# aticejiang/MLAgg-UNet

Hardware: AMD Instinct MI355X
Metric: images/sec (train step) MLAgg-UNet-2D 256x256 bs10 (higher is better)
Workload: dtype f32; 1 GPU; nnUNetTrainer_MLAgg_2D_dt_MS train step, AbdomenMRI-shaped 256x256x1, 14 classes, attention variant B (BASELINE.json configs[1]); batch_per_gpu=10, global_batch=10, parallelism=dp1, launch=eager, miopen=tuned find-db (mlagg-unet_amd/miopen_db), library_gemm=TunableOp table (mlagg-unet_amd/gemm_db), tuning off

## Files before the change

### mlagg-unet_amd/csrc/api.hip

```cpp
#include <hip/hip_runtime.h>

#include <mutex>
#include <vector>

#include "mlagg_hip.h"
#include "prof.h"

namespace mlagg_prof {

int g_selected = -1;

namespace {
struct Rec {
    int id;
    hipEvent_t start, stop;
};
std::mutex g_mu;
std::vector<Rec> g_recs;
size_t g_used = 0;
const char *const kNames[K_COUNT] = {
    "selscan_fwd_kernel<false>", "selscan_chunk_prefix", "selscan_fwd_kernel<true>", "selscan_bwd_local_kernel",
    "selscan_bwd_group_kernel", "selscan_reduce_partials", "local_attn_fwd_kernel", "local_attn_bwd_a_kernel",
    "local_attn_bwd_b_kernel", "pooled_attn_fwd_kernel", "pooled_attn_bwd1_kernel",
    "pooled_attn_bwd2_kernel", "dwconv_tiled_kernel<fwd>", "dwconv_tiled_kernel<dgrad>", "dwconv_bwd_weight_kernel", "linear weight gradient (K5w: linear_wgrad_kernel / linear_wgrad_x3_kernel + reduce)", "layernorm_fwd_kernel",
    "layernorm_bwd_kernel", "dwconv_nchw_fwd_kernel", "dwconv_nchw_bwd (data+weight+reduce)",
    "cross_scan_kernel<false>", "cross_scan_kernel<true>", "gate_fwd_kernel", "gate_bwd_kernel",
    "linear forward + data gradient (K5: linear_x3_kernel on weight images; MLAGG_K5_V2=0: linear_lp_kernel<true, MODE> / linear_mfma_kernel<true>)", "linear data gradient (K5: linear_mfma_kernel<false> / linear_lp_kernel<false, MODE>)", "row_scale_kernel", "dice_ce_stats_kernel", "dice_ce_grad_kernel", "transpose_tile_kernel", "bias gradient (plane_sum / column_sum)", "plane_norm_fwd_kernel", "plane_norm_bwd_kernel", "adamw (sumsq + update)", "flash_fwd_kernel", "flash_bwd (dq + dk/dv)", "channel_epilogue (bias + residual + GELU)",
    "sel1_fwd_kernel<2, false>", "sel1_fwd_kernel<2, true>", "sel1_bwd_local_kernel<2>", "sel1_bwd_kernel<2>",
    "sel1_fwd_kernel<R != 2, false>", "sel1_fwd_kernel<R != 2, true>", "sel1_bwd_local_kernel<R != 2>", "sel1_bwd_kernel<R != 2>",
    "sel1_prefix_kernel", "sel1 reductions (step partials + per-chunk rows)",
    "volume_pad_kernel (+ guard fill)", "conv_wgrad_taps_kernel", "conv_wgrad_reduce_kernel", "conv_taps_kernel (forward / data gradient)",
    "gelu_pool (forward + backward)", "conv1x1 (forward / data gradient / weight gradient)",
    "conv3x3 (forward / data gradient / weight gradient, incl. weight image and reduce)",
    "tok_fwd_kernel<false>", "tok_fwd_kernel<true>", "tok_bwd_local_kernel", "tok_bwd_group_kernel",
    "sw_gather_kernel", "sw_fold_kernel", "sw_finalize_kernel", "resample_linear_kernel", "export_kernel",
    "pp_box_kernel", "pp_stats_kernel (+ final)", "pp_normalize_kernel", "pp_minmax_kernel", "pp_cubic_kernel", "pp_gather_kernel",
    "cc_local_kernel", "cc_merge_kernel", "cc_compress_kernel", "cc_size_kernel", "cc_max_kernel", "cc_write_kernel",
    "sf_stats_kernel (+ init)", "sf_codes_kernel", "sf_zpass_kernel", "sf_ypass_kernel", "sf_xpass_kernel", "sf_sum_kernel",
    "aug3d_resample_kernel", "pt_seg_crop_kernel", "pt_seg_resize_kernel", "pt_rank_count_kernel (+ scan)", "pt_rank_select_kernel",
    "cl_local_kernel", "cl_merge_kernel", "cl_compress_kernel", "cl_flag_kernel", "cl_scan (count + offsets + apply)", "cl_rewrite_kernel",
    "cl_overlap_kernel", "cl_match_kernel", "ens_mean_kernel", "label_confusion_kernel", "dice_bce_stats_kernel", "dice_bce_grad_kernel",
    "aug3d_planar_kernel", "sw_gather_onehot_kernel"};
}

void record(int id, hipStream_t st, bool begin)
{
    std::lock_guard<std::mutex> lk(g_mu);
    if (begin) {
        if (g_used == g_recs.size()) {
            Rec r{id, nullptr, nullptr};
            if (hipEventCreate(&r.start) != hipSuccess || hipEventCreate(&r.stop) != hipSuccess) return;
            g_recs.push_back(r);
        }
        g_recs[g_used].id = id;
        (void)hipEventRecord(g_recs[g_used].start, st);
        ++g_used;
    } else if (g_used > 0) {
        (void)hipEventRecord(g_recs[g_used - 1].stop, st);
    }
}

}

extern "C" const char *mlagg_version(void) { return "mlagg_hip 0.1 (gfx950)"; }

extern "C" const char *mlagg_error_string(int code)
{
    switch (code) {
    case 0: return "success";
    case MLAGG_E_UNSUPPORTED: return "unsupported shape for the gfx950 kernels";
    case MLAGG_E_NULLPTR: return "required pointer argument is NULL";
    case MLAGG_E_WORKSPACE: return "workspace too small";
    default: return code > 0 ? hipGetErrorString(static_cast<hipError_t>(code)) : "unknown mlagg error";
    }
}

extern "C" int mlagg_profile_kernel_count(void) { return mlagg_prof::K_COUNT; }

extern "C" const char *mlagg_profile_kernel_name(int id)
{
    return (id >= 0 && id < mlagg_prof::K_COUNT) ? mlagg_prof::kNames[id] : "?";
}

extern "C" int mlagg_profile_select(int id)
{
    if (id < -2 || id >= mlagg_prof::K_COUNT) return MLAGG_E_UNSUPPORTED;
    mlagg_prof::g_selected = id;
    return 0;
}

extern "C" int mlagg_profile_collect(double *ms, int *counts)
{
    using namespace mlagg_prof;
    if (!ms || !counts) return MLAGG_E_NULLPTR;
    std::lock_guard<std::mutex> lk(g_mu);
    for (int i = 0; i < K_COUNT; ++i) { ms[i] = 0.0; counts[i] = 0; }
    for (size_t i = 0; i < g_used; ++i) {
        float t = 0.f;
        if (hipEventSynchronize(g_recs[i].stop) != hipSuccess) continue;
        if (hipEventElapsedTime(&t, g_recs[i].start, g_recs[i].stop) != hipSuccess) continue;
        ms[g_recs[i].id] += t;
        counts[g_recs[i].id] += 1;
    }
    g_used = 0;
    return 0;
}
```

### mlagg-unet_amd/csrc/local_attn.hip

```cpp
#include <hip/hip_runtime.h>

#include "mlagg_hip.h"
#include "prof.h"
#include "internal.h"
#include "reduce.h"

namespace {

constexpr int HD2 = 48;
constexpr int PER = 12;
constexpr int TILE = 8;
constexpr float RMS_EPS = 1e-5f;
constexpr float OUT_GAIN = 0.2f;
constexpr int WS_PER_UNIT = 76;

struct Geom {
    int batch, H, W, nh, d;
    int q_stride, kv_stride, out_stride;
    float scale;
};

__device__ __forceinline__ void load12(const float *__restrict__ p, float (&x)[PER])
{
    const float4 a = *reinterpret_cast<const float4 *>(p);
    const float4 b = *reinterpret_cast<const float4 *>(p + 4);
    const float4 c = *reinterpret_cast<const float4 *>(p + 8);
    x[0] = a.x; x[1] = a.y; x[2] = a.z; x[3] = a.w;
    x[4] = b.x; x[5] = b.y; x[6] = b.z; x[7] = b.w;
    x[8] = c.x; x[9] = c.y; x[10] = c.z; x[11] = c.w;
}

__device__ __forceinline__ void store12(float *__restrict__ p, const float (&x)[PER])
{
    *reinterpret_cast<float4 *>(p) = make_float4(x[0], x[1], x[2], x[3]);
    *reinterpret_cast<float4 *>(p + 4) = make_float4(x[4], x[5], x[6], x[7]);
    *reinterpret_cast<float4 *>(p + 8) = make_float4(x[8], x[9], x[10], x[11]);
}

struct Unit {
    int b, h, y, x, r;
    bool act;
};

__device__ __forceinline__ Unit unit_id(const Geom &g)
{
    Unit u;
    const int tiles_x = (g.W + TILE - 1) / TILE;
    const int ty = blockIdx.x / tiles_x, tx = blockIdx.x - ty * tiles_x;
    const int lu = threadIdx.x >> 2;
    u.r = threadIdx.x & 3;
    u.y = ty * TILE + (lu >> 3);
    u.x = tx * TILE + (lu & 7);
    u.h = blockIdx.y;
    u.b = blockIdx.z;
    u.act = u.y < g.H && u.x < g.W;
    return u;
}

__device__ __forceinline__ void window_softmax(const float (&l)[9], unsigned valid, float (&s)[9])
{
    float m = -3.0e38f;
#pragma unroll
    for (int j = 0; j < 9; ++j)
        if ((valid >> j) & 1) m = fmaxf(m, l[j]);
    float z = 0.f;
#pragma unroll
    for (int j = 0; j < 9; ++j) {
        s[j] = ((valid >> j) & 1) ? __expf(l[j] - m) : 0.f;
        z += s[j];
    }
    const float iz = 1.f / z;
#pragma unroll
    for (int j = 0; j < 9; ++j) s[j] *= iz;
}

struct Front {
    float s[9];
    float other[9];
    float Aw[9];
    float o[PER];
    float rstd;
    unsigned valid;
};

__device__ __forceinline__ void front_half(const Geom &g, const Unit &u, const float *__restrict__ q,
                                           const float *__restrict__ kv, float lam, Front &f)
{
    const int N = g.H * g.W;
    const size_t tok = (size_t)u.b * N + (size_t)u.y * g.W + u.x;
    float qv[PER];
    load12(q + tok * g.q_stride + u.h * HD2 + PER * u.r, qv);
    float lg[9];
    f.valid = 0;
#pragma unroll
    for (int j = 0; j < 9; ++j) {
        const int yy = u.y + j / 3 - 1, xx = u.x + j % 3 - 1;
        const bool in = yy >= 0 && yy < g.H && xx >= 0 && xx < g.W;
        float p = 0.f;
        if (in) {
            f.valid |= 1u << j;
            float kx[PER];
            load12(kv + ((size_t)u.b * N + (size_t)yy * g.W + xx) * g.kv_stride + u.h * HD2 + PER * u.r, kx);
#pragma unroll
            for (int e = 0; e < PER; ++e) p += qv[e] * kx[e];
        }
        lg[j] = (p + dpp_quad_xor1(p)) * g.scale;
    }
    window_softmax(lg, f.valid, f.s);
#pragma unroll
    for (int j = 0; j < 9; ++j) {
        f.other[j] = dpp_quad_xor2(f.s[j]);
        f.Aw[j] = u.r < 2 ? f.s[j] - lam * f.other[j] : f.other[j] - lam * f.s[j];
    }
#pragma unroll
    for (int e = 0; e < PER; ++e) f.o[e] = 0.f;
}

__device__ __forceinline__ void stage_lepe(float (*swt)[HD2], const float *__restrict__ lepe_w, int head)
{
    for (int i = threadIdx.x; i < 9 * HD2; i += blockDim.x) {
        const int c = i / 9, j = i - 9 * c;
        swt[j][c] = lepe_w[(head * HD2 + c) * 9 + j];
    }
    __syncthreads();
}

__global__ void __launch_bounds__(256)
local_attn_fwd_kernel(const float *__restrict__ q, const float *__restrict__ kv, const float *__restrict__ lamp,
                      const float *__restrict__ subln_w, const float *__restrict__ lepe_w,
                      const float *__restrict__ lepe_b, float *__restrict__ out, Geom g)
{
    __shared__ float swt[9][HD2];
    stage_lepe(swt, lepe_w, blockIdx.y);
    const Unit u = unit_id(g);
    if (!u.act) return;
    const float lam = lamp[0];
    const int N = g.H * g.W;
    Front f;
    front_half(g, u, q, kv, lam, f);
    const int cbase = u.h * HD2 + PER * u.r;
    float lp[PER];
#pragma unroll
    for (int e = 0; e < PER; ++e) lp[e] = lepe_b[cbase + e];
#pragma unroll
    for (int j = 0; j < 9; ++j) {
        if (!((f.valid >> j) & 1)) continue;
        const int yy = u.y + j / 3 - 1, xx = u.x + j % 3 - 1;
        float vx[PER], wj[PER];
        load12(kv + ((size_t)u.b * N + (size_t)yy * g.W + xx) * g.kv_stride + g.d + cbase, vx);
        load12(&swt[j][PER * u.r], wj);
#pragma unroll
        for (int e = 0; e < PER; ++e) {
            f.o[e] += f.Aw[j] * vx[e];
            lp[e] += wj[e] * vx[e];
        }
    }
    float ss = 0.f;
#pragma unroll
    for (int e = 0; e < PER; ++e) ss += f.o[e] * f.o[e];
    const float rstd = rsqrtf(quad_sum(ss) * (1.f / HD2) + RMS_EPS);
    float res[PER];
#pragma unroll
    for (int e = 0; e < PER; ++e) res[e] = OUT_GAIN * subln_w[PER * u.r + e] * f.o[e] * rstd + lp[e];
    store12(out + ((size_t)u.b * N + (size_t)u.y * g.W + u.x) * g.out_stride + cbase, res);
}

__global__ void __launch_bounds__(256)
local_attn_bwd_a_kernel(const float *__restrict__ q, const float *__restrict__ kv, const float *__restrict__ lamp,
                        const float *__restrict__ subln_w, const float *__restrict__ dout, int dout_stride,
                        float *__restrict__ dq, int dq_stride, float *__restrict__ ws, float *__restrict__ pgrad, Geom g)
{
    __shared__ float red[4][4][PER + 1];
    __syncthreads();
    const Unit u = unit_id(g);
    const float lam = lamp[0];
    const int N = g.H * g.W;
    float dw[PER];
#pragma unroll
    for (int e = 0; e < PER; ++e) dw[e] = 0.f;
    float dl_acc = 0.f;
    if (u.act) {
        Front f;
        front_half(g, u, q, kv, lam, f);
        const int cbase = u.h * HD2 + PER * u.r;
        const size_t tok = (size_t)u.b * N + (size_t)u.y * g.W + u.x;
        float vj[9][PER];
#pragma unroll
        for (int j = 0; j < 9; ++j) {
            const int yy = u.y + j / 3 - 1, xx = u.x + j % 3 - 1;
            if ((f.valid >> j) & 1) {
                load12(kv + ((size_t)u.b * N + (size_t)yy * g.W + xx) * g.kv_stride + g.d + cbase, vj[j]);
            } else {
#pragma unroll
                for (int e = 0; e < PER; ++e) vj[j][e] = 0.f;
            }
#pragma unroll
            for (int e = 0; e < PER; ++e) f.o[e] += f.Aw[j] * vj[j][e];
        }
        float ss = 0.f;
#pragma unroll
        for (int e = 0; e < PER; ++e) ss += f.o[e] * f.o[e];
        const float rstd = rsqrtf(quad_sum(ss) * (1.f / HD2) + RMS_EPS);
        float dy[PER], dO[PER];
        load12(dout + tok * dout_stride + cbase, dy);
        float dot = 0.f;
#pragma unroll
        for (int e = 0; e < PER; ++e) {
            const float wdy = subln_w[PER * u.r + e] * dy[e];
            dot += wdy * f.o[e];
            dw[e] = OUT_GAIN * dy[e] * f.o[e] * rstd;
        }
        dot = quad_sum(dot) * (1.f / HD2) * rstd * rstd;
#pragma unroll
        for (int e = 0; e < PER; ++e)
            dO[e] = OUT_GAIN * rstd * (subln_w[PER * u.r + e] * dy[e] - f.o[e] * dot);
        float dA[9];
#pragma unroll
        for (int j = 0; j < 9; ++j) {
            float p = 0.f;
#pragma unroll
            for (int e = 0; e < PER; ++e) p += dO[e] * vj[j][e];
            dA[j] = quad_sum(p);
        }
        float dsum = 0.f, dlm = 0.f;
        float ds[9];
#pragma unroll
        for (int j = 0; j < 9; ++j) {
            ds[j] = u.r < 2 ? dA[j] : -lam * dA[j];
            dsum += ds[j] * f.s[j];
            if (u.r == 2) dlm -= dA[j] * f.s[j];
        }
        dl_acc = dlm;
        float dlg[9];
#pragma unroll
        for (int j = 0; j < 9; ++j) dlg[j] = f.s[j] * (ds[j] - dsum) * g.scale;
        float dqv[PER];
#pragma unroll
        for (int e = 0; e < PER; ++e) dqv[e] = 0.f;
#pragma unroll
        for (int j = 0; j < 9; ++j) {
            if (!((f.valid >> j) & 1)) continue;
            const int yy = u.y + j / 3 - 1, xx = u.x + j % 3 - 1;
            float kx[PER];
            load12(kv + ((size_t)u.b * N + (size_t)yy * g.W + xx) * g.kv_stride + u.h * HD2 + PER * u.r, kx);
#pragma unroll
            for (int e = 0; e < PER; ++e) dqv[e] += dlg[j] * kx[e];
        }
        store12(dq + tok * dq_stride + cbase, dqv);
        float *wrow = ws + (tok * g.nh + u.h) * WS_PER_UNIT;
        if (u.r == 0) {
#pragma unroll
            for (int j = 0; j < 9; ++j) { wrow[j] = f.Aw[j]; wrow[9 + j] = dlg[j]; }
        }
        if (u.r == 2) {
#pragma unroll
            for (int j = 0; j < 9; ++j) wrow[18 + j] = dlg[j];
        }
        store12(wrow + 28 + PER * u.r, dO);
    }
#pragma unroll
    for (int e = 0; e < PER; ++e) {
        float v = dw[e];
#pragma unroll
        for (int off = 4; off < 64; off <<= 1) v += __shfl_xor(v, off, 64);
        if ((threadIdx.x & 63) < 4) red[threadIdx.x >> 6][threadIdx.x & 3][e] = v;
    }
    {
        float v = dl_acc;
#pragma unroll
        for (int off = 1; off < 64; off <<= 1) v += __shfl_xor(v, off, 64);
        if ((threadIdx.x & 63) == 0) red[threadIdx.x >> 6][0][PER] = v;
    }
    __syncthreads();
    float *prow = pgrad + ((size_t)(blockIdx.z * gridDim.y + blockIdx.y) * gridDim.x + blockIdx.x) * (4 * PER + 1);
    if (threadIdx.x < 4 * PER) {
        const int r = threadIdx.x / PER, e = threadIdx.x % PER;
        prow[threadIdx.x] = (red[0][r][e] + red[1][r][e]) + (red[2][r][e] + red[3][r][e]);
    }
    if (threadIdx.x == 63) prow[4 * PER] = (red[0][0][PER] + red[1][0][PER]) + (red[2][0][PER] + red[3][0][PER]);
}

__global__ void __launch_bounds__(256)
local_attn_bwd_b_kernel(const float *__restrict__ q, const float *__restrict__ lepe_w,
                        const float *__restrict__ dout, int dout_stride, const float *__restrict__ ws,
                        float *__restrict__ dkv, int dkv_stride, Geom g)
{
    __shared__ float swt[9][HD2];
    stage_lepe(swt, lepe_w, blockIdx.y);
    const Unit u = unit_id(g);
    if (!u.act) return;
    const int N = g.H * g.W;
    const int cbase = u.h * HD2 + PER * u.r;
    const size_t tok = (size_t)u.b * N + (size_t)u.y * g.W + u.x;
    float dk[PER], dv[PER];
#pragma unroll
    for (int e = 0; e < PER; ++e) { dk[e] = 0.f; dv[e] = 0.f; }
#pragma unroll
    for (int jj = 0; jj < 9; ++jj) {
        const int yy = u.y + jj / 3 - 1, xx = u.x + jj % 3 - 1;
        if (!(yy >= 0 && yy < g.H && xx >= 0 && xx < g.W)) continue;
        const int jw = 8 - jj;
        const size_t ti = (size_t)u.b * N + (size_t)yy * g.W + xx;
        const float *wrow = ws + (ti * g.nh + u.h) * WS_PER_UNIT;
        const float Ai = wrow[jw];
        const float dli = wrow[(u.r < 2 ? 9 : 18) + jw];
        float dOi[PER], qi[PER], dyi[PER], wj[PER];
        load12(wrow + 28 + PER * u.r, dOi);
        load12(q + ti * g.q_stride + cbase, qi);
        load12(dout + ti * dout_stride + cbase, dyi);
        load12(&swt[jw][PER * u.r], wj);
#pragma unroll
        for (int e = 0; e < PER; ++e) {
            dv[e] += Ai * dOi[e] + wj[e] * dyi[e];
            dk[e] += dli * qi[e];
        }
    }
    store12(dkv + tok * dkv_stride + cbase, dk);
    store12(dkv + tok * dkv_stride + g.d + cbase, dv);
}

int make_geom(Geom &g, int batch, int H, int W, int nh, int qs, int kvs, int outs, float scale)
{
    if (batch <= 0 || H <= 0 || W <= 0 || nh <= 0 || batch > 65535 || nh > 65535) return MLAGG_E_UNSUPPORTED;
    g.batch = batch; g.H = H; g.W = W; g.nh = nh; g.d = nh * HD2;
    g.q_stride = qs; g.kv_stride = kvs; g.out_stride = outs; g.scale = scale;
    if (qs < g.d || kvs < 2 * g.d || (qs & 3) || (kvs & 3)) return MLAGG_E_UNSUPPORTED;
    return 0;
}

dim3 tile_grid(const Geom &g)
{
    return dim3(((g.W + TILE - 1) / TILE) * ((g.H + TILE - 1) / TILE), g.nh, g.batch);
}

}

extern "C" int mlagg_local_attn_fwd(const float *q, int q_stride, const float *kv, int kv_stride,
                                    const float *lam, const float *subln_w, const float *lepe_w,
                                    const float *lepe_b, float *out, int out_stride, int batch, int H, int W,
                                    int nh, float scale, void *stream)
{
    if (!q || !kv || !lam || !subln_w || !lepe_w || !lepe_b || !out) return MLAGG_E_NULLPTR;
    Geom g;
    if (int rc = make_geom(g, batch, H, W, nh, q_stride, kv_stride, out_stride, scale)) return rc;
    if (out_stride < g.d || (out_stride & 3)) return MLAGG_E_UNSUPPORTED;
    hipStream_t st = static_cast<hipStream_t>(stream);
    { MLAGG_TIMED(K_LOCAL_FWD, st); hipLaunchKernelGGL(local_attn_fwd_kernel, tile_grid(g), dim3(256), 0, st, q, kv, lam, subln_w, lepe_w, lepe_b,
                       out, g); }
    return (int)hipGetLastError();
}

extern "C" size_t mlagg_local_attn_bwd_workspace_floats(int batch, int H, int W, int nh)
{
    const size_t tiles = (size_t)((W + TILE - 1) / TILE) * ((H + TILE - 1) / TILE) * nh * batch;
    return (size_t)batch * H * W * nh * WS_PER_UNIT + mlagg_internal::dwconv_wgrad_workspace_floats(batch, H, W, nh * HD2) +
           tiles * (4 * PER + 1);
}

extern "C" int mlagg_local_attn_bwd(const float *q, int q_stride, const float *kv, int kv_stride,
                                    const float *lam, const float *subln_w, const float *lepe_w,
                                    const float *dout, int dout_stride, float *dq, int dq_stride, float *dkv,
                                    int dkv_stride, float *dlam, float *dsubln_w, float *dlepe_w,
                                    float *dlepe_b, float *workspace, int batch, int H, int W, int nh,
                                    float scale, void *stream)
{
    if (!q || !kv || !lam || !subln_w || !lepe_w || !dout || !dq || !dkv || !dlam || !dsubln_w || !dlepe_w ||
        !dlepe_b || !workspace)
        return MLAGG_E_NULLPTR;
    Geom g;
    if (int rc = make_geom(g, batch, H, W, nh, q_stride, kv_stride, dout_stride, scale)) return rc;
    if (dout_stride < g.d || (dout_stride & 3) || dq_stride < g.d || (dq_stride & 3) || dkv_stride < 2 * g.d ||
        (dkv_stride & 3))
        return MLAGG_E_UNSUPPORTED;
    hipStream_t st = static_cast<hipStream_t>(stream);
    const dim3 tg = tile_grid(g);
    const int nwg = (int)(tg.x * tg.y * tg.z);
    float *pgrad = workspace + (size_t)batch * H * W * nh * WS_PER_UNIT + mlagg_internal::dwconv_wgrad_workspace_floats(batch, H, W, g.d);
    { MLAGG_TIMED(K_LOCAL_BWD_A, st); hipLaunchKernelGGL(local_attn_bwd_a_kernel, tg, dim3(256), 0, st, q, kv, lam, subln_w, dout,
                       dout_stride, dq, dq_stride, workspace, pgrad, g);
      hipLaunchKernelGGL(mlagg_internal::column_sum_split_kernel<0>, dim3(1), dim3(1024), 0, st, pgrad, nwg, 4 * PER + 1, 4 * PER + 1,
                         4 * PER, dsubln_w, dlam); }
    { MLAGG_TIMED(K_LOCAL_BWD_B, st); hipLaunchKernelGGL(local_attn_bwd_b_kernel, tile_grid(g), dim3(256), 0, st, q, lepe_w, dout, dout_stride,
                       workspace, dkv, dkv_stride, g); }
    mlagg_internal::dwconv_wgrad_launch(kv + g.d, kv_stride, dout, dout_stride, nullptr, dlepe_w, dlepe_b,
                                        workspace + (size_t)batch * H * W * nh * WS_PER_UNIT, batch, H, W, g.d, 0, st);
    return (int)hipGetLastError();
}
```

### mlagg-unet_amd/csrc/prof.h

```cpp
#pragma once
#include <hip/hip_runtime.h>

namespace mlagg_prof {

enum KernelId {
    K_SELSCAN_FWD_LOCAL = 0, K_SELSCAN_PREFIX, K_SELSCAN_FWD_FINAL, K_SELSCAN_BWD_LOCAL, K_SELSCAN_BWD,
    K_SELSCAN_REDUCE, K_LOCAL_FWD, K_LOCAL_BWD_A, K_LOCAL_BWD_B, K_POOLED_FWD,
    K_POOLED_BWD1, K_POOLED_BWD2, K_DWCONV_FWD, K_DWCONV_BWD_DATA, K_DWCONV_BWD_WEIGHT, K_LINEAR_WGRAD, K_LAYERNORM_FWD, K_LAYERNORM_BWD, K_DWCONV_NCHW_FWD, K_DWCONV_NCHW_BWD, K_CROSS_SCAN, K_CROSS_MERGE, K_GATE_FWD, K_GATE_BWD, K_LINEAR_FWD, K_LINEAR_DGRAD, K_ROW_SCALE, K_LOSS_STATS, K_LOSS_GRAD, K_TRANSPOSE, K_BIAS_GRAD, K_PLANE_NORM_FWD, K_PLANE_NORM_BWD, K_ADAMW, K_FLASH_FWD, K_FLASH_BWD, K_CHANNEL_EPI,
    K_SEL1_FWD_LOCAL_R2, K_SEL1_FWD_FINAL_R2, K_SEL1_BWD_LOCAL_R2, K_SEL1_BWD_R2, K_SEL1_FWD_LOCAL, K_SEL1_FWD_FINAL, K_SEL1_BWD_LOCAL,
    K_SEL1_BWD, K_SEL1_PREFIX, K_SEL1_REDUCE, K_CONV_PAD, K_CONV_WGRAD, K_CONV_WGRAD_REDUCE, K_CONV_TAPS, K_GELU_POOL, K_CONV1X1, K_CONV3X3, K_TOK_FWD_LOCAL, K_TOK_FWD_FINAL, K_TOK_BWD_LOCAL, K_TOK_BWD_GROUP, K_SW_GATHER, K_SW_FOLD, K_SW_FINALIZE, K_RESAMPLE_LINEAR, K_EXPORT_SEG, K_PP_BOX, K_PP_STATS, K_PP_NORMALIZE, K_PP_MINMAX, K_PP_CUBIC, K_PP_GATHER, K_CC_LOCAL, K_CC_MERGE, K_CC_COMPRESS, K_CC_SIZE, K_CC_MAX, K_CC_WRITE, K_SF_STATS, K_SF_CODES, K_SF_ZPASS, K_SF_YPASS, K_SF_XPASS, K_SF_SUM, K_AUG3D_RESAMPLE, K_PT_SEG_CROP, K_PT_SEG_RESIZE, K_PT_RANK_COUNTS, K_PT_RANK_SELECT,
    K_CL_LOCAL, K_CL_MERGE, K_CL_COMPRESS, K_CL_FLAG, K_CL_SCAN, K_CL_REWRITE, K_CL_OVERLAP, K_CL_MATCH,
    K_ENS_MEAN, K_LABEL_CONFUSION, K_REGION_LOSS_STATS, K_REGION_LOSS_GRAD, K_AUG3D_PLANAR, K_SW_GATHER_ONEHOT, K_COUNT
};

extern int g_selected;
void record(int id, hipStream_t st, bool begin);

struct Scope {
    int id;
    hipStream_t st;
    bool on;
    Scope(int id_, hipStream_t st_) : id(id_), st(st_), on(g_selected == -2 || g_selected == id_)
    {
        if (on) record(id, st, true);
    }
    ~Scope()
    {
        if (on) record(id, st, false);
    }
};

}

#define MLAGG_TIMED(id, st) mlagg_prof::Scope mlagg_prof_scope_##id(mlagg_prof::id, st)
```

### mlagg-unet_amd/profiling.py

```python
import ctypes

from . import _lib


def _names():
    lib = _lib.lib()
    return [lib.mlagg_profile_kernel_name(i).decode() for i in range(lib.mlagg_profile_kernel_count())]


def select_all():
    _lib.check(_lib.lib().mlagg_profile_select(-2), "mlagg_profile_select")


def select(name):
    idx = -1 if name is None else _names().index(name)
    _lib.check(_lib.lib().mlagg_profile_select(idx), "mlagg_profile_select")


def collect():
    lib = _lib.lib()
    n = lib.mlagg_profile_kernel_count()
    ms = (ctypes.c_double * n)()
    cnt = (ctypes.c_int * n)()
    _lib.check(lib.mlagg_profile_collect(ms, cnt), "mlagg_profile_collect")
    return {nm: {"ms": ms[i], "count": cnt[i]} for i, nm in enumerate(_names()) if cnt[i] > 0}


def algorithmic_bytes(kernel, batch, img):
    H, W = img
    n0 = (H // 2) * (W // 2)
    l_cat = sum(n0 >> (2 * i) for i in range(4))
    D, N, G, R = 384, 16, 4, 3
    scan = {
        "selscan_fwd_kernel<false>": 4 * l_cat * (D + G * R + G * N),
        "selscan_fwd_kernel<true>": 4 * l_cat * (2 * D + G * R + 2 * G * N),
        "selscan_bwd_local_kernel": 4 * l_cat * (D + G * R + G * N),
        "selscan_bwd_group_kernel": 4 * l_cat * (3 * D + 2 * G * R + 4 * G * N),
        "tok_fwd_kernel<false>": 4 * l_cat * G * (96 + 4 + N),
        "tok_fwd_kernel<true>": 4 * l_cat * G * (96 + 36 + 96),
        "tok_bwd_local_kernel": 4 * l_cat * G * (96 + 4 + N),
        "tok_bwd_group_kernel": 4 * l_cat * G * (3 * 96 + 2 * 36),
    }
    if kernel in scan:
        return scan[kernel] * batch
    dn = sum(48 * n0 / 2 ** i for i in range(4)) / 4
    per_module = {
        "local_attn_fwd_kernel": 16 * dn,
        "local_attn_bwd_a_kernel": 20 * dn,
        "local_attn_bwd_b_kernel": 16 * dn,
        "pooled_attn_fwd_kernel": 8 * dn,
        "pooled_attn_bwd1_kernel": 16 * dn,
        "pooled_attn_bwd2_kernel": 8 * dn,
    }
    return int(per_module.get(kernel, 0) * batch)


def algorithmic_bytes_sel1(kernel, batch, tokens, C=64, K=12, R=2):
    par = 4 * (3 + R)
    per_token = {
        "sel1_fwd_kernel<2, false>": K * (4 * C + par),
        "sel1_fwd_kernel<2, true>": K * (4 * C + par) + 4 * C,
        "sel1_bwd_local_kernel<2>": K * (4 * C + par),
        "sel1_bwd_kernel<2>": K * (8 * C + par + 4 * (2 + R)) + 4 * C,
    }
    return int(per_token.get(kernel, 0)) * tokens * batch
```

Measured before the change: 284.4 images/sec.

## Fuse local attention backward passes via LDS halo recompute

Merges the two local-attention backward kernels into one tiled kernel. Each workgroup recomputes the front half for a one-pixel halo ring around its 8x8 tile and parks the per-token attention weights, logit grads, dO, q and dy in LDS, so dk/dv can be gathered without the global workspace round trip. A two-level reduction is added for the per-tile parameter-gradient partials when there are many tiles. The cost is redundant halo recomputation, roughly 36 extra units per 64, plus large LDS use that may limit occupancy.

New measurement: 287.2 images/sec, median of 6. No clear change (+1.0%).

```diff
diff --git a/mlagg-unet_amd/csrc/api.hip b/mlagg-unet_amd/csrc/api.hip
--- a/mlagg-unet_amd/csrc/api.hip
+++ b/mlagg-unet_amd/csrc/api.hip
@@ -20,8 +20,8 @@
 size_t g_used = 0;
 const char *const kNames[K_COUNT] = {
     "selscan_fwd_kernel<false>", "selscan_chunk_prefix", "selscan_fwd_kernel<true>", "selscan_bwd_local_kernel",
-    "selscan_bwd_group_kernel", "selscan_reduce_partials", "local_attn_fwd_kernel", "local_attn_bwd_a_kernel",
-    "local_attn_bwd_b_kernel", "pooled_attn_fwd_kernel", "pooled_attn_bwd1_kernel",
+    "selscan_bwd_group_kernel", "selscan_reduce_partials", "local_attn_fwd_kernel", "local_attn_bwd_kernel",
+    "pooled_attn_fwd_kernel", "pooled_attn_bwd1_kernel",
     "pooled_attn_bwd2_kernel", "dwconv_tiled_kernel<fwd>", "dwconv_tiled_kernel<dgrad>", "dwconv_bwd_weight_kernel", "linear weight gradient (K5w: linear_wgrad_kernel / linear_wgrad_x3_kernel + reduce)", "layernorm_fwd_kernel",
     "layernorm_bwd_kernel", "dwconv_nchw_fwd_kernel", "dwconv_nchw_bwd (data+weight+reduce)",
     "cross_scan_kernel<false>", "cross_scan_kernel<true>", "gate_fwd_kernel", "gate_bwd_kernel",
diff --git a/mlagg-unet_amd/csrc/local_attn.hip b/mlagg-unet_amd/csrc/local_attn.hip
--- a/mlagg-unet_amd/csrc/local_attn.hip
+++ b/mlagg-unet_amd/csrc/local_attn.hip
@@ -12,7 +12,7 @@
 constexpr int TILE = 8;
 constexpr float RMS_EPS = 1e-5f;
 constexpr float OUT_GAIN = 0.2f;
-constexpr int WS_PER_UNIT = 76;
+constexpr int WS_FLOOR_PER_UNIT = 76;
 
 struct Geom {
     int batch, H, W, nh, d;
@@ -79,6 +79,7 @@
     float other[9];
     float Aw[9];
     float o[PER];
+    float q[PER];
     float rstd;
     unsigned valid;
 };
@@ -88,8 +89,7 @@
 {
     const int N = g.H * g.W;
     const size_t tok = (size_t)u.b * N + (size_t)u.y * g.W + u.x;
-    float qv[PER];
-    load12(q + tok * g.q_stride + u.h * HD2 + PER * u.r, qv);
+    load12(q + tok * g.q_stride + u.h * HD2 + PER * u.r, f.q);
     float lg[9];
     f.valid = 0;
 #pragma unroll
@@ -102,7 +102,7 @@
             float kx[PER];
             load12(kv + ((size_t)u.b * N + (size_t)yy * g.W + xx) * g.kv_stride + u.h * HD2 + PER * u.r, kx);
 #pragma unroll
-            for (int e = 0; e < PER; ++e) p += qv[e] * kx[e];
+            for (int e = 0; e < PER; ++e) p += f.q[e] * kx[e];
         }
         lg[j] = (p + dpp_quad_xor1(p)) * g.scale;
     }
@@ -165,24 +165,56 @@
     store12(out + ((size_t)u.b * N + (size_t)u.y * g.W + u.x) * g.out_stride + cbase, res);
 }
 
-__global__ void __launch_bounds__(256)
-local_attn_bwd_a_kernel(const float *__restrict__ q, const float *__restrict__ kv, const float *__restrict__ lamp,
-                        const float *__restrict__ subln_w, const float *__restrict__ dout, int dout_stride,
-                        float *__restrict__ dq, int dq_stride, float *__restrict__ ws, float *__restrict__ pgrad, Geom g)
-{
-    __shared__ float red[4][4][PER + 1];
-    __syncthreads();
-    const Unit u = unit_id(g);
+constexpr int PARK = 80;
+
+struct BwdTile {
+    static constexpr int HW = TILE + 2, HH = TILE + 2, NH = HW * HH;
+    static constexpr int THREADS = TILE * TILE * 4, WAVES = THREADS / 64;
+    static constexpr int RING = 2 * HW + 2 * TILE;
+    static constexpr size_t LDS_BYTES = sizeof(float) * (NH * (PARK + 2 * HD2) + 9 * HD2 + WAVES * 4 * (PER + 1));
+};
+
+__global__ void __launch_bounds__(BwdTile::THREADS)
+local_attn_bwd_kernel(const float *__restrict__ q, const float *__restrict__ kv, const float *__restrict__ lamp,
+                      const float *__restrict__ subln_w, const float *__restrict__ lepe_w, const float *__restrict__ dout,
+                      int dout_stride, float *__restrict__ dq, int dq_stride, float *__restrict__ dkv, int dkv_stride,
+                      float *__restrict__ pgrad, Geom g)
+{
+    using T = BwdTile;
+    extern __shared__ float4 lds4[];
+    float *park = reinterpret_cast<float *>(lds4);
+    float *sq = park + T::NH * PARK;
+    float *sdy = sq + T::NH * HD2;
+    float (*swt)[HD2] = reinterpret_cast<float (*)[HD2]>(sdy + T::NH * HD2);
+    float (*red)[4][PER + 1] = reinterpret_cast<float (*)[4][PER + 1]>(sdy + T::NH * HD2 + 9 * HD2);
+    stage_lepe(swt, lepe_w, blockIdx.y);
+    const int tiles_x = (g.W + TILE - 1) / TILE;
+    const int ty = blockIdx.x / tiles_x, tx = blockIdx.x - ty * tiles_x;
+    const int lu = threadIdx.x >> 2, r = threadIdx.x & 3;
     const float lam = lamp[0];
     const int N = g.H * g.W;
+    const int cbase = blockIdx.y * HD2 + PER * r;
     float dw[PER];
 #pragma unroll
     for (int e = 0; e < PER; ++e) dw[e] = 0.f;
     float dl_acc = 0.f;
-    if (u.act) {
+#pragma unroll 1
+    for (int pass = 0; pass < 2; ++pass) {
+        int hy, hx;
+        if (pass == 0) { hy = lu / TILE + 1; hx = lu % TILE + 1; }
+        else if (lu < T::HW) { hy = 0; hx = lu; }
+        else if (lu < 2 * T::HW) { hy = T::HH - 1; hx = lu - T::HW; }
+        else if (lu < T::RING) { hy = 1 + ((lu - 2 * T::HW) >> 1); hx = ((lu - 2 * T::HW) & 1) ? T::HW - 1 : 0; }
+        else break;
+        Unit u;
+        u.b = blockIdx.z; u.h = blockIdx.y; u.r = r;
+        u.y = ty * TILE + hy - 1;
+        u.x = tx * TILE + hx - 1;
+        u.act = u.y >= 0 && u.y < g.H && u.x >= 0 && u.x < g.W;
+        if (!u.act) continue;
+        const int hidx = hy * T::HW + hx;
         Front f;
         front_half(g, u, q, kv, lam, f);
-        const int cbase = u.h * HD2 + PER * u.r;
         const size_t tok = (size_t)u.b * N + (size_t)u.y * g.W + u.x;
         float vj[9][PER];
 #pragma unroll
@@ -206,14 +238,14 @@
         float dot = 0.f;
 #pragma unroll
         for (int e = 0; e < PER; ++e) {
-            const float wdy = subln_w[PER * u.r + e] * dy[e];
+            const float wdy = subln_w[PER * r + e] * dy[e];
             dot += wdy * f.o[e];
-            dw[e] = OUT_GAIN * dy[e] * f.o[e] * rstd;
+            if (pass == 0) dw[e] = OUT_GAIN * dy[e] * f.o[e] * rstd;
         }
         dot = quad_sum(dot) * (1.f / HD2) * rstd * rstd;
 #pragma unroll
         for (int e = 0; e < PER; ++e)
-            dO[e] = OUT_GAIN * rstd * (subln_w[PER * u.r + e] * dy[e] - f.o[e] * dot);
+            dO[e] = OUT_GAIN * rstd * (subln_w[PER * r + e] * dy[e] - f.o[e] * dot);
         float dA[9];
 #pragma unroll
         for (int j = 0; j < 9; ++j) {
@@ -226,37 +258,41 @@
         float ds[9];
 #pragma unroll
         for (int j = 0; j < 9; ++j) {
-            ds[j] = u.r < 2 ? dA[j] : -lam * dA[j];
+            ds[j] = r < 2 ? dA[j] : -lam * dA[j];
             dsum += ds[j] * f.s[j];
-            if (u.r == 2) dlm -= dA[j] * f.s[j];
-        }
-        dl_acc = dlm;
+            if (r == 2) dlm -= dA[j] * f.s[j];
+        }
         float dlg[9];
 #pragma unroll
         for (int j = 0; j < 9; ++j) dlg[j] = f.s[j] * (ds[j] - dsum) * g.scale;
-        float dqv[PER];
-#pragma unroll
-        for (int e = 0; e < PER; ++e) dqv[e] = 0.f;
-#pragma unroll
-        for (int j = 0; j < 9; ++j) {
-            if (!((f.valid >> j) & 1)) continue;
-            const int yy = u.y + j / 3 - 1, xx = u.x + j % 3 - 1;
-            float kx[PER];
-            load12(kv + ((size_t)u.b * N + (size_t)yy * g.W + xx) * g.kv_stride + u.h * HD2 + PER * u.r, kx);
-#pragma unroll
-            for (int e = 0; e < PER; ++e) dqv[e] += dlg[j] * kx[e];
-        }
-        store12(dq + tok * dq_stride + cbase, dqv);
-        float *wrow = ws + (tok * g.nh + u.h) * WS_PER_UNIT;
-        if (u.r == 0) {
-#pragma unroll
-            for (int j = 0; j < 9; ++j) { wrow[j] = f.Aw[j]; wrow[9 + j] = dlg[j]; }
-        }
-        if (u.r == 2) {
-#pragma unroll
-            for (int j = 0; j < 9; ++j) wrow[18 + j] = dlg[j];
-        }
-        store12(wrow + 28 + PER * u.r, dO);
+        if (pass == 0) {
+            dl_acc = dlm;
+            float dqv[PER];
+#pragma unroll
+            for (int e = 0; e < PER; ++e) dqv[e] = 0.f;
+#pragma unroll
+            for (int j = 0; j < 9; ++j) {
+                if (!((f.valid >> j) & 1)) continue;
+                const int yy = u.y + j / 3 - 1, xx = u.x + j % 3 - 1;
+                float kx[PER];
+                load12(kv + ((size_t)u.b * N + (size_t)yy * g.W + xx) * g.kv_stride + u.h * HD2 + PER * r, kx);
+#pragma unroll
+                for (int e = 0; e < PER; ++e) dqv[e] += dlg[j] * kx[e];
+            }
+            store12(dq + tok * dq_stride + cbase, dqv);
+        }
+        float *prow = park + hidx * PARK;
+        if (r == 0) {
+#pragma unroll
+            for (int j = 0; j < 9; ++j) { prow[j] = f.Aw[j]; prow[9 + j] = dlg[j]; }
+        }
+        if (r == 2) {
+#pragma unroll
+            for (int j = 0; j < 9; ++j) prow[18 + j] = dlg[j];
+        }
+        store12(prow + 28 + PER * r, dO);
+        store12(sq + hidx * HD2 + PER * r, f.q);
+        store12(sdy + hidx * HD2 + PER * r, dy);
     }
 #pragma unroll
     for (int e = 0; e < PER; ++e) {
@@ -272,52 +308,65 @@
         if ((threadIdx.x & 63) == 0) red[threadIdx.x >> 6][0][PER] = v;
     }
     __syncthreads();
-    float *prow = pgrad + ((size_t)(blockIdx.z * gridDim.y + blockIdx.y) * gridDim.x + blockIdx.x) * (4 * PER + 1);
-    if (threadIdx.x < 4 * PER) {
-        const int r = threadIdx.x / PER, e = threadIdx.x % PER;
-        prow[threadIdx.x] = (red[0][r][e] + red[1][r][e]) + (red[2][r][e] + red[3][r][e]);
-    }
-    if (threadIdx.x == 63) prow[4 * PER] = (red[0][0][PER] + red[1][0][PER]) + (red[2][0][PER] + red[3][0][PER]);
-}
-
-__global__ void __launch_bounds__(256)
-local_attn_bwd_b_kernel(const float *__restrict__ q, const float *__restrict__ lepe_w,
-                        const float *__restrict__ dout, int dout_stride, const float *__restrict__ ws,
-                        float *__restrict__ dkv, int dkv_stride, Geom g)
-{
-    __shared__ float swt[9][HD2];
-    stage_lepe(swt, lepe_w, blockIdx.y);
-    const Unit u = unit_id(g);
-    if (!u.act) return;
-    const int N = g.H * g.W;
-    const int cbase = u.h * HD2 + PER * u.r;
-    const size_t tok = (size_t)u.b * N + (size_t)u.y * g.W + u.x;
+    float *wgrow = pgrad + ((size_t)(blockIdx.z * gridDim.y + blockIdx.y) * gridDim.x + blockIdx.x) * (4 * PER + 1);
+    if (threadIdx.x < 4 * PER + 1) {
+        const int rr = threadIdx.x < 4 * PER ? threadIdx.x / PER : 0, e = threadIdx.x < 4 * PER ? threadIdx.x % PER : PER;
+        float s = (red[0][rr][e] + red[1][rr][e]) + (red[2][rr][e] + red[3][rr][e]);
+        wgrow[threadIdx.x] = s;
+    }
+    const int ly = lu / TILE, lx = lu % TILE;
+    const int y = ty * TILE + ly, x = tx * TILE + lx;
+    if (y >= g.H || x >= g.W) return;
     float dk[PER], dv[PER];
 #pragma unroll
     for (int e = 0; e < PER; ++e) { dk[e] = 0.f; dv[e] = 0.f; }
 #pragma unroll
     for (int jj = 0; jj < 9; ++jj) {
-        const int yy = u.y + jj / 3 - 1, xx = u.x + jj % 3 - 1;
+        const int yy = y + jj / 3 - 1, xx = x + jj % 3 - 1;
         if (!(yy >= 0 && yy < g.H && xx >= 0 && xx < g.W)) continue;
         const int jw = 8 - jj;
-        const size_t ti = (size_t)u.b * N + (size_t)yy * g.W + xx;
-        const float *wrow = ws + (ti * g.nh + u.h) * WS_PER_UNIT;
-        const float Ai = wrow[jw];
-        const float dli = wrow[(u.r < 2 ? 9 : 18) + jw];
+        const int hi = (ly + jj / 3) * T::HW + lx + jj % 3;
+        const float *prow = park + hi * PARK;
+        const float Ai = prow[jw];
+        const float dli = prow[(r < 2 ? 9 : 18) + jw];
         float dOi[PER], qi[PER], dyi[PER], wj[PER];
-        load12(wrow + 28 + PER * u.r, dOi);
-        load12(q + ti * g.q_stride + cbase, qi);
-        load12(dout + ti * dout_stride + cbase, dyi);
-        load12(&swt[jw][PER * u.r], wj);
+        load12(prow + 28 + PER * r, dOi);
+        load12(sq + hi * HD2 + PER * r, qi);
+        load12(sdy + hi * HD2 + PER * r, dyi);
+        load12(&swt[jw][PER * r], wj);
 #pragma unroll
         for (int e = 0; e < PER; ++e) {
             dv[e] += Ai * dOi[e] + wj[e] * dyi[e];
             dk[e] += dli * qi[e];
         }
     }
+    const size_t tok = (size_t)blockIdx.z * N + (size_t)y * g.W + x;
     store12(dkv + tok * dkv_stride + cbase, dk);
     store12(dkv + tok * dkv_stride + g.d + cbase, dv);
 }
+
+__global__ void __launch_bounds__(1024)
+local_attn_pgrad_rows_kernel(const float *__restrict__ part, int rows, int per, int cols, float *__restrict__ out)
+{
+    __shared__ float red[16][65];
+    const int c = threadIdx.x & 63, rg = threadIdx.x >> 6;
+    const int r0 = blockIdx.x * per, r1 = min(rows, r0 + per);
+    float s = 0.f;
+    if (c < cols)
+        for (int row = r0 + rg; row < r1; row += 16) s += part[(size_t)row * cols + c];
+    red[rg][c] = s;
+    __syncthreads();
+    if (rg == 0 && c < cols) {
+        float t = 0.f;
+#pragma unroll
+        for (int i = 0; i < 16; ++i) t += red[i][c];
+        out[(size_t)blockIdx.x * cols + c] = t;
+    }
+}
+
+constexpr int PGRAD_COLS = 4 * PER + 1;
+constexpr int PGRAD_ROWS_PER_WG = 64;
+constexpr int PGRAD_SPLIT_ABOVE = 1024;
 
 int make_geom(Geom &g, int batch, int H, int W, int nh, int qs, int kvs, int outs, float scale)
 {
@@ -353,8 +402,10 @@
 extern "C" size_t mlagg_local_attn_bwd_workspace_floats(int batch, int H, int W, int nh)
 {
     const size_t tiles = (size_t)((W + TILE - 1) / TILE) * ((H + TILE - 1) / TILE) * nh * batch;
-    return (size_t)batch * H * W * nh * WS_PER_UNIT + mlagg_internal::dwconv_wgrad_workspace_floats(batch, H, W, nh * HD2) +
-           tiles * (4 * PER + 1);
+    const size_t level1 = (tiles + PGRAD_ROWS_PER_WG - 1) / PGRAD_ROWS_PER_WG;
+    const size_t need = mlagg_internal::dwconv_wgrad_workspace_floats(batch, H, W, nh * HD2) + (tiles + level1) * PGRAD_COLS;
+    const size_t floor = (size_t)batch * H * W * nh * WS_FLOOR_PER_UNIT;
+    return need > floor ? need : floor;
 }
 
 extern "C" int mlagg_local_attn_bwd(const float *q, int q_stride, const float *kv, int kv_stride,
@@ -375,14 +426,27 @@
     hipStream_t st = static_cast<hipStream_t>(stream);
     const dim3 tg = tile_grid(g);
     const int nwg = (int)(tg.x * tg.y * tg.z);
-    float *pgrad = workspace + (size_t)batch * H * W * nh * WS_PER_UNIT + mlagg_internal::dwconv_wgrad_workspace_floats(batch, H, W, g.d);
-    { MLAGG_TIMED(K_LOCAL_BWD_A, st); hipLaunchKernelGGL(local_attn_bwd_a_kernel, tg, dim3(256), 0, st, q, kv, lam, subln_w, dout,
-                       dout_stride, dq, dq_stride, workspace, pgrad, g);
-      hipLaunchKernelGGL(mlagg_internal::column_sum_split_kernel<0>, dim3(1), dim3(1024), 0, st, pgrad, nwg, 4 * PER + 1, 4 * PER + 1,
-                         4 * PER, dsubln_w, dlam); }
-    { MLAGG_TIMED(K_LOCAL_BWD_B, st); hipLaunchKernelGGL(local_attn_bwd_b_kernel, tile_grid(g), dim3(256), 0, st, q, lepe_w, dout, dout_stride,
-                       workspace, dkv, dkv_stride, g); }
-    mlagg_internal::dwconv_wgrad_launch(kv + g.d, kv_stride, dout, dout_stride, nullptr, dlepe_w, dlepe_b,
-                                        workspace + (size_t)batch * H * W * nh * WS_PER_UNIT, batch, H, W, g.d, 0, st);
+    float *lepe_part = workspace;
+    float *pgrad = lepe_part + mlagg_internal::dwconv_wgrad_workspace_floats(batch, H, W, g.d);
+    float *pgrad1 = pgrad + (size_t)nwg * PGRAD_COLS;
+    {
+        MLAGG_TIMED(K_LOCAL_BWD, st);
+        static const int rc = mlagg_internal::allow_lds(local_attn_bwd_kernel, BwdTile::LDS_BYTES);
+        if (rc) return rc;
+        hipLaunchKernelGGL(local_attn_bwd_kernel, tg, dim3(BwdTile::THREADS), BwdTile::LDS_BYTES, st, q, kv, lam, subln_w, lepe_w, dout,
+                           dout_stride, dq, dq_stride, dkv, dkv_stride, pgrad, g);
+        const float *rows = pgrad;
+        int nrows = nwg;
+        if (nwg > PGRAD_SPLIT_ABOVE) {
+            nrows = (nwg + PGRAD_ROWS_PER_WG - 1) / PGRAD_ROWS_PER_WG;
+            hipLaunchKernelGGL(local_attn_pgrad_rows_kernel, dim3(nrows), dim3(1024), 0, st, pgrad, nwg, PGRAD_ROWS_PER_WG, PGRAD_COLS,
+                               pgrad1);
+            rows = pgrad1;
+        }
+        hipLaunchKernelGGL(mlagg_internal::column_sum_split_kernel<0>, dim3(1), dim3(1024), 0, st, rows, nrows, PGRAD_COLS, PGRAD_COLS,
+                           4 * PER, dsubln_w, dlam);
+    }
+    mlagg_internal::dwconv_wgrad_launch(kv + g.d, kv_stride, dout, dout_stride, nullptr, dlepe_w, dlepe_b, lepe_part, batch, H, W,
+                                        g.d, 0, st);
     return (int)hipGetLastError();
 }
diff --git a/mlagg-unet_amd/csrc/prof.h b/mlagg-unet_amd/csrc/prof.h
--- a/mlagg-unet_amd/csrc/prof.h
+++ b/mlagg-unet_amd/csrc/prof.h
@@ -5,7 +5,7 @@
 
 enum KernelId {
     K_SELSCAN_FWD_LOCAL = 0, K_SELSCAN_PREFIX, K_SELSCAN_FWD_FINAL, K_SELSCAN_BWD_LOCAL, K_SELSCAN_BWD,
-    K_SELSCAN_REDUCE, K_LOCAL_FWD, K_LOCAL_BWD_A, K_LOCAL_BWD_B, K_POOLED_FWD,
+    K_SELSCAN_REDUCE, K_LOCAL_FWD, K_LOCAL_BWD, K_POOLED_FWD,
     K_POOLED_BWD1, K_POOLED_BWD2, K_DWCONV_FWD, K_DWCONV_BWD_DATA, K_DWCONV_BWD_WEIGHT, K_LINEAR_WGRAD, K_LAYERNORM_FWD, K_LAYERNORM_BWD, K_DWCONV_NCHW_FWD, K_DWCONV_NCHW_BWD, K_CROSS_SCAN, K_CROSS_MERGE, K_GATE_FWD, K_GATE_BWD, K_LINEAR_FWD, K_LINEAR_DGRAD, K_ROW_SCALE, K_LOSS_STATS, K_LOSS_GRAD, K_TRANSPOSE, K_BIAS_GRAD, K_PLANE_NORM_FWD, K_PLANE_NORM_BWD, K_ADAMW, K_FLASH_FWD, K_FLASH_BWD, K_CHANNEL_EPI,
     K_SEL1_FWD_LOCAL_R2, K_SEL1_FWD_FINAL_R2, K_SEL1_BWD_LOCAL_R2, K_SEL1_BWD_R2, K_SEL1_FWD_LOCAL, K_SEL1_FWD_FINAL, K_SEL1_BWD_LOCAL,
     K_SEL1_BWD, K_SEL1_PREFIX, K_SEL1_REDUCE, K_CONV_PAD, K_CONV_WGRAD, K_CONV_WGRAD_REDUCE, K_CONV_TAPS, K_GELU_POOL, K_CONV1X1, K_CONV3X3, K_TOK_FWD_LOCAL, K_TOK_FWD_FINAL, K_TOK_BWD_LOCAL, K_TOK_BWD_GROUP, K_SW_GATHER, K_SW_FOLD, K_SW_FINALIZE, K_RESAMPLE_LINEAR, K_EXPORT_SEG, K_PP_BOX, K_PP_STATS, K_PP_NORMALIZE, K_PP_MINMAX, K_PP_CUBIC, K_PP_GATHER, K_CC_LOCAL, K_CC_MERGE, K_CC_COMPRESS, K_CC_SIZE, K_CC_MAX, K_CC_WRITE, K_SF_STATS, K_SF_CODES, K_SF_ZPASS, K_SF_YPASS, K_SF_XPASS, K_SF_SUM, K_AUG3D_RESAMPLE, K_PT_SEG_CROP, K_PT_SEG_RESIZE, K_PT_RANK_COUNTS, K_PT_RANK_SELECT,
diff --git a/mlagg-unet_amd/profiling.py b/mlagg-unet_amd/profiling.py
--- a/mlagg-unet_amd/profiling.py
+++ b/mlagg-unet_amd/profiling.py
@@ -46,8 +46,7 @@
     dn = sum(48 * n0 / 2 ** i for i in range(4)) / 4
     per_module = {
         "local_attn_fwd_kernel": 16 * dn,
-        "local_attn_bwd_a_kernel": 20 * dn,
-        "local_attn_bwd_b_kernel": 16 * dn,
+        "local_attn_bwd_kernel": 28 * dn,
         "pooled_attn_fwd_kernel": 8 * dn,
         "pooled_attn_bwd1_kernel": 16 * dn,
         "pooled_attn_bwd2_kernel": 8 * dn,
```
